# metarank/metarank

Hardware: AMD Instinct MI355X
Metric: ranked items/sec (feature assembly + 500-tree LambdaMART + ordering), Ranklens-shaped 100-item requests (higher is better)
Workload: dtype f64

## Files before the change

### metarank_amd/csrc/capi.cpp

```cpp
#include <cmath>
#include <cstddef>
#include <cstdlib>
#include <cstring>
#include <mutex>
#include <set>
#include <thread>
#include <utility>

#include "runtime.hpp"

namespace mrk {

static thread_local std::string g_last_error;
void set_last_error(const std::string &msg) { g_last_error = msg; }

static Switches read_switches() {
  Switches s;
  auto flag = [](const char *name, bool dflt) { const char *e = getenv(name); return e ? atoi(e) != 0 : dflt; };
  auto num = [](const char *name, int dflt) { const char *e = getenv(name); return e ? atoi(e) : dflt; };
  s.rank_fused = flag("MRK_RANK_FUSED", true);
  s.rank_cells = flag("MRK_RANK_CELLS", true);
  if (const char *e = getenv("MRK_SCORER")) s.scorer_walk = !strcmp(e, "walk");
  if (const char *e = getenv("MRK_FUSED_THREADS")) s.fused_threads = std::min(256, std::max(64, atoi(e) / 64 * 64));
  { const int fs = num("MRK_FUSED_SPLIT", 0); s.fused_split = fs == 1 || fs == 2 || fs == 4 ? fs : 0; }
// ... 25 lines not shown
  s.jit_shipped = flag("MRK_JIT_SHIPPED", true);
  if (const char *d = getenv("MRK_JIT_DEFINES")) s.jit_defines = d; else s.jit_defines.clear();
  s.thr_stage = flag("MRK_THR_STAGE", true);
  s.fused_lds_min = std::max(0, num("MRK_FUSED_LDS_MIN", 0));
  if (const char *d = getenv("MRK_JIT_CACHE_DIR")) s.jit_cache_dir = d;
  else if (const char *x = getenv("XDG_CACHE_HOME")) s.jit_cache_dir = std::string(x) + "/mrk_jit";
  else if (const char *h = getenv("HOME")) s.jit_cache_dir = std::string(h) + "/.cache/mrk_jit";
  if (s.jit_cache_dir == "off") s.jit_cache_dir.clear();
  s.big_sort_cap = num("MRK_BIG_SORT_CAP", 4096);
  s.big_sort_tile = num("MRK_BIG_SORT_TILE", 0);
  s.big_sort_bucket = num("MRK_BIG_SORT_BUCKET", 0);
  s.jit_prepass = flag("MRK_JIT_PREPASS", true);
  s.qs_split = num("MRK_QS_SPLIT", -1);
  s.qs_kernel = num("MRK_QS_KERNEL", 1);
  s.qs_byte = flag("MRK_QS_BYTE", true);
  s.qs_r = num("MRK_QS_R", 2);
  s.walk_tile = num("MRK_WALK_TILE", 0);
  s.encoder_graph = flag("MRK_ENCODER_GRAPH", false);
  s.encoder_skinny = num("MRK_ENCODER_SKINNY", 15);
  s.encoder_packed = flag("MRK_ENCODER_PACKED", true);
  s.encoder_f32_mfma = flag("MRK_ENCODER_F32_MFMA", true);
  return s;
}
static Switches &switches_storage() {
  static Switches s = read_switches();
  return s;
}
const Switches &switches() { return switches_storage(); }
void reload_switches() { switches_storage() = read_switches(); }

// ... 492 lines not shown
```

### metarank_amd/csrc/capi_rank.cpp

```cpp
#include <algorithm>
#include <atomic>
#include <chrono>
#include <condition_variable>
#include <cstring>
#include <thread>

#include <linux/futex.h>
#include <sched.h>
#include <sys/prctl.h>
#include <sys/syscall.h>
#include <time.h>
#include <unistd.h>

#include <cstdlib>

#include "features.hpp"
#include "jit.hpp"
#include "launch_shape.hpp"
#include "qs_device.hpp"
#include "rank.hpp"
#include "runtime.hpp"

namespace mrk {

// ... 64 lines not shown
}

}

using namespace mrk;

struct mrk_batch {
  mrk_ctx *ctx = nullptr;
  const Program *prog = nullptr;
  int n_req = 0, total_items = 0;
  std::mutex bmu;
  DevBuf d_in, d_prep_out, d_arena, d_matrix;
  hipStream_t stream = nullptr;
  hipStream_t s() const { return stream ? stream : ctx->stream; }
  DevBuf d_out;
  size_t out_order_off = 0, out_status_off = 0, out_bytes = 0;
  PinBuf h_out;
  bool fetch_enqueued = false;
  bool direct_out = false;
  DevBuf d_cells;
  DevBuf d_sort;
  DevBuf d_norm_order;
  DevBuf d_gather;
  DevBuf d_gather_status;
  struct BigReq { int r, n_items, item_begin; };
  std::vector<BigReq> big;
  PinBuf h_in;
  HostBatch hb;
  DevBuf d_ids;
  PinBuf h_ids;
  BatchDev view{};
// ... 117 lines not shown
  uint8_t *h = b.h_in.as<uint8_t>();
  auto put = [&](size_t o, const void *src, size_t bytes) { if (bytes) memcpy(h + o, src, bytes); };
  put(o_reqs, hb.reqs.data(), hb.reqs.size() * sizeof(ReqDev));
  put(o_consts, hb.consts.data(), hb.consts.size() * 8);
  put(o_irf, hb.irf.data(), hb.irf.size() * 4);
  put(o_ov, hb.overrides.data(), hb.overrides.size() * sizeof(Override));
  put(o_prep, hb.prep_out.data(), hb.prep_out.size() * sizeof(PrepOut));
  if (!hb.device_ids) {
    put(o_slot, hb.item_slot.data(), (size_t)T * 4);
    put(o_ireq, hb.item_req.data(), (size_t)T * 4);
  }
  MRK_HIP(hipMemcpyAsync(b.d_in.p, h, up_bytes, hipMemcpyHostToDevice, b.s()));
  uint8_t *d = b.d_in.as<uint8_t>();
  const size_t score_slots = (size_t)T + 256 * QS_TILE_ROWS;
  b.out_order_off = align_up(score_slots * 8, 256);
  b.out_status_off = align_up(b.out_order_off + std::max<size_t>(T, 1) * 4, 256);
  b.out_bytes = b.out_status_off + 2 * std::max<size_t>(n_req, 1) * 4;
  b.d_out.reserve(b.out_bytes);
  int32_t *d_load_status = (int32_t *)(b.d_out.as<uint8_t>() + b.out_status_off) + std::max(n_req, 1);
  MRK_HIP(hipMemsetAsync(d_load_status, 0, std::max<size_t>(n_req, 1) * 4, b.s()));
  if (hb.device_ids && T > 0) {
    const size_t off_bytes = ((size_t)T + 1) * 4;
    const size_t id_bytes = ids->offsets[T];
    if (id_bytes > ids->bytes_len || ids->bytes_len > 0xffffffffull)
      throw StatusError(MRK_ERR_INVALID_ARG, "mrk_item_ids: the last offset passes bytes_len (or bytes_len >= 4 GiB)");
    const size_t o_bytes = align_up(off_bytes, 256);
    b.d_ids.reserve(o_bytes + std::max<size_t>(id_bytes, 1));
    const void *src_off = ids->offsets, *src_bytes = ids->bytes;
    const bool own_staging = (const void *)ids->offsets == (const void *)b.h_ids.p;
    if (!own_staging && (!is_pinned_host(ids->offsets) || !is_pinned_host(ids->bytes))) {
      b.h_ids.reserve(o_bytes + std::max<size_t>(id_bytes, 1));
// ... 15 lines not shown
  v.total_items = T;
  v.item_lo = 0;
  v.item_hi = T;
  v.item_slot = (const int32_t *)(d + o_slot);
  v.item_req = (const uint32_t *)(d + o_ireq);
  v.consts = (const double *)(d + o_consts);
  v.irf = (const int32_t *)(d + o_irf);
  v.overrides = (const Override *)(d + o_ov);
  v.n_overrides = (int)hb.overrides.size();
  v.prep_out = (PrepOut *)(d + o_prep);
  v.arena = (unsigned long long *)b.d_arena.p;
  v.status = (int32_t *)(b.d_out.as<uint8_t>() + b.out_status_off);
  v.matrix = (double *)b.d_matrix.p;
  v.scores = (double *)b.d_out.p;
  v.order = (int32_t *)(b.d_out.as<uint8_t>() + b.out_order_off);
  b.h_status.assign(n_req, 0);
  b.ran = false;
  b.matrix_valid = false;
  b.fetch_enqueued = false;
  b.big.clear();
  size_t big_bytes = 0;
  for (int r = 0; r < n_req; ++r)
    if (hb.reqs[r].n_items > SORT_MAX_ITEMS) {
      b.big.push_back({r, hb.reqs[r].n_items, (int)hb.reqs[r].item_begin});
      big_bytes = std::max(big_bytes, big_sort_scratch_bytes(hb.reqs[r].n_items));
    }
  if (big_bytes) b.d_sort.reserve(big_bytes);
  uint32_t vals = 1;
  while ((int)vals < hb.max_doubles) vals <<= 1;
  b.fused_entries = (uint32_t)std::max<uint64_t>(hb.max_req_entries, 1);
// ... 95 lines not shown
  b.fetch_enqueued = false;
  b.direct_out = false;
  if (one) {
    b.h_out.reserve(b.out_bytes);
    uint8_t *h = b.h_out.as<uint8_t>();
    const OneOut out{(double *)h, (int32_t *)(h + b.out_order_off), (int32_t *)(h + b.out_status_off),
                     (const int32_t *)(b.d_out.as<uint8_t>() + b.out_status_off) + std::max(b.n_req, 1), std::max(b.n_req, 1)};
    b.view.item_lo = 0;
    b.view.item_hi = b.total_items;
    launch_rank_one(ctx, st, pd, b.view, b.fused_entries, b.fused_vals, b.fused_threads, b.fused_split, qs_device_view(model), qs_forest_view(model), out, f64, jit_fn);
    b.matrix_valid = false;
    b.direct_out = true;
    b.ran = true;
    return;
  }
  MRK_HIP(hipMemsetAsync(b.view.status, 0, std::max<size_t>(b.n_req, 1) * 4, b.s()));
  b.view.item_lo = whole_matrix ? 0 : lo;
  b.view.item_hi = whole_matrix ? b.total_items : hi;
  if (fused_score) {
    const QsDev q = qs_device_view(model);
    b.d_cells.reserve(std::max<size_t>((size_t)b.n_req * q.n_views * QS_TILE_ROWS * 2, 16));
    launch_rank_fused_score(ctx, st, pd, b.view, b.fused_entries, b.fused_vals, b.fused_threads, q, qs_forest_view(model), b.d_cells.as<uint16_t>(), f64, jit_fn);
    b.matrix_valid = false;
    b.ran = true;
    return;
  }
  if (cells) {
    const QsDev q = qs_device_view(model);
    const size_t tile_bytes = (size_t)q.n_views * QS_TILE_ROWS * 2;
    const size_t n_tiles = ((size_t)b.total_items + QS_TILE_ROWS - 1) / QS_TILE_ROWS;
    b.d_cells.reserve(std::max<size_t>(n_tiles * tile_bytes, 16));
    if (hi % QS_TILE_ROWS && tile_bytes)
      MRK_HIP(hipMemsetAsync(b.d_cells.as<uint8_t>() + (size_t)(hi / QS_TILE_ROWS) * tile_bytes, 0, tile_bytes, b.s()));
    if (b.fused_ok) {
      launch_rank_fused(ctx, st, pd, b.view, b.fused_entries, b.fused_vals, b.fused_threads, b.fused_split, b.fused_slices, &q, b.d_cells.as<uint16_t>(), f64, jit_fn,
                        sig && sig->ok ? (size_t)sig->rt_total * 8 : 0);
    } else {
      launch_prepass(ctx, st, pd, b.view, b.fused_entries, jit_prep_fn);
      launch_assemble_cells(ctx, st, pd, b.view, q, b.d_cells.as<uint16_t>(), f64, jit_fn, b.fused_entries, jit_rt_fn, jit_rt_fn ? model->qs_sig.rt_total : 0u);
    }
    b.matrix_valid = false;
    launch_score_qs_cells(ctx, model, b.d_cells.as<uint16_t>() + (size_t)(lo / QS_TILE_ROWS) * (tile_bytes / 2), rows, b.view.scores + lo);
  } else {
    assemble_matrix(b, st, pd, jit_fn);
    b.matrix_valid = whole_matrix || (lo == 0 && hi == b.total_items);
    if (model && rows > 0) {
      launch_score_batch(ctx, model, b.view.matrix + (size_t)lo * pd.dim, rows, pd.dim, b.view.scores + lo, b.view.status, b.view.item_req + lo);
    } else if (rows > 0) {
      MRK_HIP(hipMemsetAsync(b.view.scores + lo, 0, (size_t)rows * 8, b.s()));
    }
  }
  b.view.item_lo = 0;
  b.view.item_hi = b.total_items;
  if (sort) sort_batch(b);
  b.ran = true;
}

// ... 1331 lines not shown
```

### metarank_amd/csrc/rank.hip

```cpp
#include <hip/hip_runtime.h>

#include <cstdint>
#include <mutex>
#include <utility>

#include "rank_device.hpp"
#include "sort_device.hpp"
#include "runtime.hpp"

namespace mrk {

namespace {

__global__ void __launch_bounds__(PREP_THREADS)
prepass_kernel(StoreDev st, ProgramDev prog, BatchDev b, uint32_t lds_entries) { prepass_body(st, prog, b, lds_entries); }

__global__ void __launch_bounds__(ASM_THREADS)
assemble_kernel(StoreDev st, ProgramDev prog, BatchDev b) {
  const int gi0 = b.item_lo + blockIdx.x * ASM_THREADS + threadIdx.x;
  const bool active = gi0 < b.item_hi;
  if (!__any(active)) return;
  const int gi = active ? gi0 : b.item_hi - 1;
  const int r = (int)b.item_req[gi];
  const ReqDev rq = b.reqs[r];
// ... 46 lines not shown

template <bool F64>
__global__ void override_cells_kernel(BatchDev b, QsDev q, uint16_t *cells) {
  const int i = blockIdx.x * blockDim.x + threadIdx.x;
  if (i >= b.n_overrides) return;
  const Override o = b.overrides[i];
  if ((int)o.item < b.item_lo || (int)o.item >= b.item_hi) return;
  if ((int)o.col >= q.n_feats) return;
  const QsFeature ft = q.feats[o.col];
  uint16_t *d = cells + (size_t)(o.item / QS_TILE_ROWS) * q.n_views * QS_TILE_ROWS + (o.item % QS_TILE_ROWS);
  const bool ok = qs_bin_column<F64>(o.value, ft, q.views, q.thr, [d](uint32_t view, uint32_t cell) { d[view * QS_TILE_ROWS] = (uint16_t)cell; });
  if (!ok) atomicOr(&b.status[b.item_req[o.item]], 32);
}

constexpr int SORT_THREADS = 256;
constexpr int SORT_COUNT_MAX = 256;

__global__ void __launch_bounds__(SORT_THREADS)
sort_kernel(BatchDev b, int cap) {
  extern __shared__ __align__(16) unsigned long long sort_smem[];
  unsigned long long *s_key = sort_smem;
  int *s_idx = (int *)(sort_smem + cap);
  const int r = blockIdx.x;
  const int tid = threadIdx.x;
  const ReqDev rq = b.reqs[r];
  const int n = rq.n_items;
  if (n <= 0 || n > SORT_MAX_ITEMS) return;
  if (n <= SORT_COUNT_MAX) {
    for (int i = tid; i < n; i += SORT_THREADS) s_key[i] = sort_key(b.scores[rq.item_begin + i]);
    __syncthreads();
    for (int i = tid; i < n; i += SORT_THREADS) {
      const unsigned long long mine = s_key[i];
      int before = 0;
      for (int j = 0; j < n; ++j) {
        const unsigned long long kj = s_key[j];
        before += (kj < mine || (kj == mine && j < i)) ? 1 : 0;
      }
      b.order[rq.item_begin + before] = i;
    }
    return;
  }
  int p2 = 1;
  while (p2 < n) p2 <<= 1;
  for (int i = tid; i < p2; i += SORT_THREADS) {
    s_key[i] = i < n ? sort_key(b.scores[rq.item_begin + i]) : ~0ull;
    s_idx[i] = i < n ? i : 0x7fffffff;
  }
  __syncthreads();
  for (int k = 2; k <= p2; k <<= 1) {
    for (int j = k >> 1; j > 0; j >>= 1) {
      for (int p = tid; p < p2 / 2; p += SORT_THREADS) {
        const int i = ((p & ~(j - 1)) << 1) | (p & (j - 1)), ixj = i | j;
        const unsigned long long ka = s_key[i], kb = s_key[ixj];
        const int ia = s_idx[i], ib = s_idx[ixj];
// ... 328 lines not shown
```

### metarank_amd/csrc/rank.hpp

```cpp
#pragma once
#include "device_types.hpp"

namespace mrk {

enum OpKind : int32_t {
  OP_SCALAR_DOUBLE = 0,
  OP_SCALAR_BOOL = 1,
  OP_VECTOR = 2,
  OP_STRING_INDEX = 3,
  OP_STRING_ONEHOT = 4,
  OP_COUNTER = 5,
  OP_WINDOW = 6,
  OP_RATE = 7,
  OP_INTERACTED = 8,
  OP_DIVERSITY = 9,
  OP_ITEM_AGE = 10,
  OP_CONST = 11,
  OP_FILL_NAN = 12,
  OP_BIENCODER = 13,
};

enum RateMode : int32_t { RATE_ITEM = 0, RATE_ITEM_FIELD = 1, RATE_RANKING_FIELD = 2 };
enum NormMode : int32_t { NORM_NOOP = 0, NORM_MINMAX = 1, NORM_POSITION = 2 };

// ... 72 lines not shown
  int32_t n_req;
  int32_t total_items;
  int32_t item_lo, item_hi;
  const int32_t *item_slot;
  const uint32_t *item_req;
  const double *consts;
  const int32_t *irf;
  const Override *overrides;
  int32_t n_overrides;
  PrepOut *prep_out;
  unsigned long long *arena;
  int32_t *status;
  double *matrix;
  double *scores;
  int32_t *order;
};

constexpr int PREP_MAX_VALUES = 4096;
struct OneOut {
  double *scores;
  int32_t *order;
  int32_t *status;
  const int32_t *load_status;
  int32_t n_req_pad;
};

struct ServeCtl {
  uint32_t seq;
  uint32_t stop;
  uint32_t ack;
// ... 7 lines not shown
  ServeCtl *ctl;
  const uint8_t *in_host;
  uint8_t *in_dev;
  OneOut out;
};
constexpr int SERVE_GANG = 8;
struct ServeGangDev {
  const ServeSlotDev *slots;
  unsigned long long *clock;
  uint32_t launch_id, pad;
  unsigned long long idle_ticks;
  unsigned long long life_ticks;
};

constexpr int SORT_MAX_ITEMS = 4096;

}
```

### metarank_amd/csrc/rank_device.hpp

```cpp
#pragma once
#include <hip/hip_runtime.h>

#include "qs_device.hpp"
#include "rank.hpp"
#include "sort_device.hpp"
#include "table_device.hpp"
#include "wave_device.hpp"

#ifdef MRK_PHASE_CLOCKS
__device__ unsigned long long mrk_phase_clocks[64];
#define MRK_PHASE(prev, acc)                                                   \
  do {                                                                         \
    const unsigned long long t_ = clock64();                                   \
    (acc) += t_ - (prev);                                                      \
    (prev) = t_;                                                               \
  } while (0)
#else
#define MRK_PHASE(prev, acc) do { } while (0)
#endif

namespace mrk {

namespace {

// ... 1509 lines not shown
  const uint8_t *irec = record(st, SC_ITEM, islot);
  constexpr int NP = prog_item_pieces<Prog>(0);
  if constexpr (NP > 0 && NP <= REC_MAX_PIECES) {
    const RegRec<NP> ir = load_record_regs<NP>(irec);
    assemble_item_rec<SPLIT>(st, prog, b, gi, r, rq, tab_base, tab_sub, pos, sink, islot, ir, og, G);
  } else {
    const PtrRec ir{irec};
    assemble_item_rec<SPLIT>(st, prog, b, gi, r, rq, tab_base, tab_sub, pos, sink, islot, ir, og, G);
  }
}


template <bool SPLIT, typename Prog, typename SinkMaker>
__device__ __forceinline__ void rank_fused_body(const StoreDev &st, const Prog &prog, const BatchDev &b, uint32_t tab_entries,
                                                int vals_cap, uint32_t thr_cap, int mode, const SinkMaker &make_sink, uint32_t lds_skip = 0,
                                                const double *rt_src = nullptr, uint32_t rt_doubles = 0, int blk = -1) {
  const int op_split = SPLIT ? ((mode & 255) > 1 ? (mode & 255) : 1) : 1;
  const int slices = SPLIT ? (((mode >> 8) & 255) > 1 ? ((mode >> 8) & 255) : 1) : 1;
  extern __shared__ __align__(16) uint8_t smem_base[];
  uint8_t *smem = smem_base + lds_skip;
  unsigned long long *s_tab = (unsigned long long *)smem;
  double *s_vals = (double *)(smem + (size_t)tab_entries * 8);
  PrepOut *s_po = (PrepOut *)(smem + (size_t)tab_entries * 8 + (size_t)vals_cap * 8);
  int *s_int = (int *)(s_po + FUSED_MAX_PREP);
  const size_t thr_at = ((size_t)((uint8_t *)(s_int + PREP_INTS) - smem) + 15) & ~(size_t)15;
  qs_lds_double *s_thr_all = (qs_lds_double *)(smem + thr_at);
  qs_lds_double *s_thr = s_thr_all + (size_t)(threadIdx.x >> 6) * 2 * thr_cap;
  const int bid = blk < 0 ? (int)blockIdx.x : blk;
  const int r = bid / slices, sl = bid % slices;
  const ReqDev rq = b.reqs[r];
  if (rq.item_begin >= b.item_hi || rq.item_begin + rq.n_items <= b.item_lo) return;
  const int item_lanes = (int)blockDim.x / op_split;
  const int per = ((rq.n_items + slices - 1) / slices + item_lanes - 1) / item_lanes * item_lanes;
  const int slice_lo = sl * per, slice_hi = min(rq.n_items, slice_lo + per);
  if (sl > 0 && slice_lo >= rq.n_items) return;
  for (int e = threadIdx.x; e < prog.n_prep; e += blockDim.x) s_po[e] = b.prep_out[(size_t)r * prog.n_prep + e];
  if (rt_doubles) {
    const uint4 *src = (const uint4 *)rt_src;
    uint4 *dst = (uint4 *)(smem + thr_at);
    for (uint32_t i = threadIdx.x; i < rt_doubles / 2; i += blockDim.x) dst[i] = src[i];
  }
  __syncthreads();
  PrepScratch sc{s_vals, vals_cap, s_int, 0ull, {0, 0, 0, 0, 0, 0}};
#ifdef MRK_PHASE_CLOCKS
  sc.clk = clock64();
#endif
  prepass_request(st, prog, b, r, rq, s_tab, (uint32_t)rq.arena_begin, s_po, sc);
  const int og = (int)threadIdx.x / item_lanes, il = (int)threadIdx.x % item_lanes;
  for (int base = slice_lo; base < slice_hi; base += item_lanes) {
    const int i = base + il;
// ... 122 lines not shown
    atomicAdd(&mrk_phase_clocks[5], clk_acc[1]);
    atomicAdd(&mrk_phase_clocks[6], 1ull);
  }
#endif
}

template <bool SPLIT = false, typename Prog>
__device__ __forceinline__ void rank_fused_matrix_body(const StoreDev &st, const Prog &prog, const BatchDev &b, uint32_t tab_entries, int vals_cap, int mode = 1) {
  rank_fused_body<SPLIT>(st, prog, b, tab_entries, vals_cap, 0u, mode,
                  [&](int gi, int, bool active, qs_lds_double *, qs_lds_double *) { return MatrixSink{b.matrix + (size_t)gi * prog.dim, active}; });
}

template <bool F64, bool SPLIT = false, typename QS = QsDyn, typename Prog>
__device__ __forceinline__ void rank_fused_cells_body(const StoreDev &st, const Prog &prog, const BatchDev &b, uint32_t tab_entries,
                                                      int vals_cap, const QsDev &q, uint16_t *cells, int mode = 1) {
  if constexpr (qs_fused_rt<QS, SPLIT>()) {
    rank_fused_body<SPLIT>(st, prog, b, tab_entries, vals_cap, qs_thr_cap<QS>(q), mode, [&](int gi, int r, bool active, qs_lds_double *, qs_lds_double *s_all) {
      return CellSinkRT<F64, QS, !SPLIT>{q, cells + (size_t)(gi / QS_TILE_ROWS) * QS::n_views * QS_TILE_ROWS + (gi % QS_TILE_ROWS), &b.status[r], s_all, active};
    }, 0u, q.thr_rt, QS::rt_total);
  } else {
    rank_fused_body<SPLIT>(st, prog, b, tab_entries, vals_cap, qs_thr_cap<QS>(q), mode, [&](int gi, int r, bool active, qs_lds_double *s_thr, qs_lds_double *) {
      return CellSink<F64, QS>{q, cells + (size_t)(gi / QS_TILE_ROWS) * qs_n_views<QS>(q) * QS_TILE_ROWS + (gi % QS_TILE_ROWS), &b.status[r], s_thr, active};
    });
  }
}

template <bool F64, typename QS = QsDyn, typename Prog>
__device__ __forceinline__ void rank_one_body(const StoreDev &st, const Prog &prog, const BatchDev &b, uint32_t tab_entries, int vals_cap,
                                              const QsDev &q, const QsForestDev &f, int mode, const OneOut &out, int blk = -1) {
  extern __shared__ __align__(16) uint8_t smem_base[];
  const int tid = threadIdx.x, nthr = blockDim.x;
  const int r = blk < 0 ? (int)blockIdx.x : blk;
  const ReqDev rq = b.reqs[r];
  const uint32_t slab_bytes = (uint32_t)qs_n_views<QS>(q) * (QS_TILE_ROWS * 2);
  for (uint32_t i = tid; i < slab_bytes / 4 + 4; i += nthr) ((uint32_t *)smem_base)[i] = 0u;
  int32_t *s_status = (int32_t *)(smem_base + slab_bytes);
  BatchDev bl = b;
  bl.status = s_status - r;
// ... 181 lines not shown
```

### metarank_amd/csrc/runtime.hpp

```cpp
#pragma once
#include <hip/hip_runtime.h>

#include <atomic>
#include <condition_variable>
#include <cstdint>
#include <map>
#include <memory>
#include <mutex>
#include <shared_mutex>
#include <stdexcept>
#include <string>
#include <vector>

#include "../../include/mrk.h"
#include "forest.hpp"

namespace mrk {

struct StatusError : std::runtime_error {
  int status;
  StatusError(int s, const std::string &m) : std::runtime_error(m), status(s) {}
};

void set_last_error(const std::string &msg);
// ... 101 lines not shown
  bool items_lds = true;
  int rank_one_max = 128;
  int split_max_req = 64;
  bool items_rt = true;
  int items_rt_threads = 0;
  bool jit_sig = true;
  bool jit_record_regs = true;
  std::string jit_cache_dir;
  int big_sort_cap = 4096;
  bool jit_prepass = true;
  int big_sort_bucket = 0;
  int big_sort_tile = 0;
  int qs_split = -1;
  int qs_kernel = 1;
  bool qs_byte = true;
  int qs_r = 2;
  int walk_tile = 0;
  bool encoder_graph = false;
  int encoder_skinny = 15;
  bool encoder_packed = true;
  bool encoder_f32_mfma = true;
};
const Switches &switches();
void reload_switches();


}

struct mrk_ctx {
  std::atomic<int> refs{1};
// ... 73 lines not shown

void lds_optin(mrk_ctx *ctx, const void *fn, int bytes = 160 * 1024);

int hw_queue_budget();

void ctx_retain(mrk_ctx *ctx);
void ctx_release(mrk_ctx *ctx);

void free_rank_state(mrk_ctx *ctx);
void comm_destroy(mrk_ctx *ctx);
void comm_allgather_f64_inplace(mrk_ctx *ctx, double *buf, size_t chunk, hipStream_t stream);
void comm_allgather_f64(mrk_ctx *ctx, const double *send, double *recv, size_t count, hipStream_t stream);
void comm_allgather_i32(mrk_ctx *ctx, const int32_t *send, int32_t *recv, size_t count, hipStream_t stream);
void unbind_encoders(mrk_ctx *ctx);

void launch_score(mrk_ctx *ctx, mrk_model *m, const double *d_x, int rows, int cols, double *d_out,
                  int *d_flag);
uint32_t score_chunk_budget();
bool launch_score_qs(mrk_ctx *ctx, mrk_model *m, const double *d_x, int rows, int cols, double *d_out, int *d_flag,
                     const uint32_t *d_row_req);
void launch_score_qs_cells(mrk_ctx *ctx, mrk_model *m, const uint16_t *d_cells, int rows, double *d_out);

}
```

### metarank_amd/csrc/score_qs.hip

```cpp
#include <hip/hip_runtime.h>

#include <algorithm>
#include <cstdint>
#include <cstdlib>

#include "launch_shape.hpp"
#include "qs_device.hpp"
#include "runtime.hpp"

namespace mrk {

QsDev qs_device_view(const mrk_model *m);

namespace {

constexpr int QS_WAVES = 4;


template <bool F64>
__global__ void __launch_bounds__(256)
qs_bin_kernel(const double *__restrict__ X, int rows, int cols, QsDev q, uint16_t *__restrict__ cells, int tile_rows,
              long long padded_rows, int *__restrict__ flag, const uint32_t *__restrict__ row_req) {
  const long long row = (long long)blockIdx.x * 256 + threadIdx.x;
  if (row >= padded_rows) return;
// ... 223 lines not shown
#pragma unroll
    for (int j = 0; j < R; ++j) { if constexpr (F64) acc64[j] += lb64[j]; else acc32[j] += lb32[j]; }
  }
#pragma unroll
  for (int j = 0; j < R; ++j) { if constexpr (F64) acc64[j] += la64[j]; else acc32[j] += la32[j]; }
  if (!odd) {
#pragma unroll
    for (int j = 0; j < R; ++j) { if constexpr (F64) acc64[j] += lb64[j]; else acc32[j] += lb32[j]; }
  }
  const long long row0 = tile * (R * 64) + (long long)lane * R;
#pragma unroll
  for (int j = 0; j < R; ++j)
    if (row0 + j < rows) out[row0 + j] = F64 ? acc64[j] : (double)acc32[j];
}

template <bool F64, int NW>
__global__ void __launch_bounds__(NW * 64)
qs_score_split_kernel(const uint32_t *__restrict__ nodes, const uint8_t *__restrict__ leaves,
                      const QsCatNode *__restrict__ cat_nodes, const uint32_t *__restrict__ cat_bits,
                      const uint16_t *__restrict__ cells, int n_trees, int V, int rows, double base,
                      double *__restrict__ out) {
  constexpr int LS = F64 ? 8 : 4;
  constexpr int TREE_LEAF_BYTES = QS_LEAVES * LS;
  constexpr int CH = 8 * NW;
  extern __shared__ __align__(16) uint8_t smem[];
  uint8_t *s_leaf = smem + (size_t)V * 256;
  uint8_t *s_idx = s_leaf + CH * TREE_LEAF_BYTES;
  const int tid = threadIdx.x;
  const int lane = tid & 63;
  const int wave = __builtin_amdgcn_readfirstlane(tid >> 6);
  const long long tile = blockIdx.x;
  {
    const uint4 *src = (const uint4 *)(cells + (size_t)tile * V * QS_TILE_ROWS);
    uint4 *dst = (uint4 *)smem;
    for (int i = tid; i < V * 16; i += NW * 64) dst[i] = src[i];
  }
// ... 42 lines not shown
      }
      const uint32_t inv = ~accn;
      const uint32_t pair = (uint32_t)__builtin_ctz(inv) | ((uint32_t)__builtin_ctz(inv >> 16) << 8);
      *(uint16_t *)(s_idx + tt * QS_TILE_ROWS + lane * 2) = (uint16_t)pair;
    }
    __syncthreads();
    if (tid < QS_TILE_ROWS) {
      for (int tt = 0; tt < nt; ++tt) {
        const uint32_t li = s_idx[tt * QS_TILE_ROWS + tid];
        if constexpr (F64) acc64 += *(const double *)(s_leaf + tt * TREE_LEAF_BYTES + li * 8);
        else acc32 += *(const float *)(s_leaf + tt * TREE_LEAF_BYTES + li * 4);
      }
    }
  }
  const long long row = tile * QS_TILE_ROWS + tid;
  if (tid < QS_TILE_ROWS && row < rows) out[row] = F64 ? acc64 : (double)acc32;
}

template <int B0>
__device__ __forceinline__ void qs_byte_block(uint32_t &acc, const uint32_t (&d)[QS_SLOTS - 1], const uint32_t (&m)[QS_SLOTS]) {
#pragma unroll
  for (int s = B0; s < B0 + 4 && s < QS_SLOTS - 1; ++s) asm("v_and_or_b32 %0, %1, %2, %0" : "+v"(acc) : "v"(d[s]), "s"(m[s]));
}

template <bool F64, int NW>
__global__ void __launch_bounds__(NW * 64)
qs_score_byte_split_kernel(const uint32_t *__restrict__ bnodes, const uint8_t *__restrict__ leaves,
                           const QsCatNode *__restrict__ cat_nodes, const uint32_t *__restrict__ cat_bits,
                           const uint16_t *__restrict__ cells, int n_trees, int V, int rows, double base,
                           double *__restrict__ out) {
  constexpr int LS = F64 ? 8 : 4;
  constexpr int TREE_LEAF_BYTES = QS_LEAVES * LS;
  constexpr int CH = 8 * NW;
  extern __shared__ __align__(16) uint8_t smem[];
  uint8_t *s_leaf = smem + (size_t)V * 256;
  uint8_t *s_idx = s_leaf + CH * TREE_LEAF_BYTES;
  const int tid = threadIdx.x;
  const int lane = tid & 63;
  const int wave = __builtin_amdgcn_readfirstlane(tid >> 6);
  const long long tile = blockIdx.x;
  const uint16_t *tile_cells = cells + (size_t)tile * V * QS_TILE_ROWS;
  {
    const uint4 *src = (const uint4 *)tile_cells;
    uint4 *dst = (uint4 *)smem;
    typedef unsigned short ushort2v __attribute__((ext_vector_type(2)));
// ... 59 lines not shown
      }
      const uint32_t inv = ~accn;
      const uint32_t pair = (uint32_t)__builtin_ctz(inv) | ((uint32_t)__builtin_ctz(inv >> 16) << 8);
      *(uint16_t *)(s_idx + tt * QS_TILE_ROWS + lane * 2) = (uint16_t)pair;
    }
    __syncthreads();
    if (tid < QS_TILE_ROWS) {
      for (int tt = 0; tt < nt; ++tt) {
        const uint32_t li = s_idx[tt * QS_TILE_ROWS + tid];
        if constexpr (F64) acc64 += *(const double *)(s_leaf + tt * TREE_LEAF_BYTES + li * 8);
        else acc32 += *(const float *)(s_leaf + tt * TREE_LEAF_BYTES + li * 4);
      }
    }
  }
  const long long row = tile * QS_TILE_ROWS + tid;
  if (tid < QS_TILE_ROWS && row < rows) out[row] = F64 ? acc64 : (double)acc32;
}

template <bool F64>
void launch_wave(mrk_ctx *ctx, mrk_model *m, const uint16_t *d_cells, int rows, double *d_out) {
  const PackedForestQS &q = m->qs;
  const int V = (int)q.views.size();
  const long long n_tiles = ((long long)rows + QS_TILE_ROWS - 1) / QS_TILE_ROWS;
  const int split_env = switches().qs_split;
  const int nw = split_env >= 0 ? split_env : scorer_waves_per_tile(n_tiles, V, F64, ctx->n_cus, QS_LEAVES, QS_TILE_ROWS);
  if (nw == 2 || nw == 4 || nw == 8 || nw == 16) {
    const size_t lds = (size_t)V * 256 + (size_t)8 * nw * (QS_LEAVES * (F64 ? 8 : 4) + QS_TILE_ROWS);
    if (lds <= 160 * 1024) {
      ScopedKernelTimer timer(ctx, "score");
      const bool byte_mode = q.byte_ok && switches().qs_byte;
#define MRK_SPLIT(NW_)                                                                                                      \
      {                                                                                                                       \
        auto sk = byte_mode ? qs_score_byte_split_kernel<F64, NW_> : qs_score_split_kernel<F64, NW_>;                        \
        lds_optin(ctx, (const void *)sk);                                                                                     \
        hipLaunchKernelGGL(sk, dim3((unsigned)n_tiles), dim3(NW_ * 64), lds, ctx->launch,                                     \
                           byte_mode ? m->d_qs_bnodes.as<uint32_t>() : m->d_qs_nodes.as<uint32_t>(),                          \
                           m->d_qs_leaves.as<uint8_t>(), m->d_qs_catnodes.as<QsCatNode>(), m->d_qs_cat.as<uint32_t>(), d_cells, \
                           q.n_trees, V, rows, m->forest.base_score, d_out);                                                  \
      }
      if (nw == 16) MRK_SPLIT(16) else if (nw == 8) MRK_SPLIT(8) else if (nw == 4) MRK_SPLIT(4) else MRK_SPLIT(2)
#undef MRK_SPLIT
      MRK_HIP(hipGetLastError());
      return;
    }
  }
  auto wk = qs_score_wave_kernel<F64>;
  lds_optin(ctx, (const void *)wk);
  const size_t lds = (size_t)V * 256;
  ScopedKernelTimer timer(ctx, "score");
  hipLaunchKernelGGL(wk, dim3((unsigned)n_tiles), dim3(64), lds, ctx->launch, m->d_qs_nodes.as<uint32_t>(),
                     m->d_qs_leaves.as<uint8_t>(), m->d_qs_catnodes.as<QsCatNode>(), m->d_qs_cat.as<uint32_t>(), d_cells,
                     q.n_trees, V, rows, m->forest.base_score, d_out);
  MRK_HIP(hipGetLastError());
}

template <bool F64, int R>
void launch_generic(mrk_ctx *ctx, mrk_model *m, const uint16_t *d_cells, int rows, double *d_out, int chunk_trees, size_t smem) {
  const PackedForestQS &q = m->qs;
  const int V = (int)q.views.size();
  const long long n_tiles = ((long long)rows + R * 64 - 1) / (R * 64);
  auto kern = qs_score_kernel<F64, R>;
  lds_optin(ctx, (const void *)kern);
  ScopedKernelTimer timer(ctx, "score");
  const int grid = (int)((n_tiles + QS_WAVES - 1) / QS_WAVES);
  hipLaunchKernelGGL(kern, dim3(grid), dim3(QS_WAVES * 64), smem, ctx->launch, m->d_qs_nodes.as<uint32_t>(),
                     m->d_qs_leaves.as<uint8_t>(), m->d_qs_catnodes.as<QsCatNode>(), m->d_qs_cat.as<uint32_t>(), d_cells,
                     q.n_trees, V, rows, n_tiles, m->forest.base_score, d_out, chunk_trees);
  MRK_HIP(hipGetLastError());
// ... 58 lines not shown
  f.cat_nodes = m->d_qs_catnodes.as<QsCatNode>();
  f.cat_bits = m->d_qs_cat.as<uint32_t>();
  f.n_trees = m->qs.n_trees;
  f.n_views = (int32_t)m->qs.views.size();
  f.base = m->forest.base_score;
  return f;
}

bool launch_score_qs(mrk_ctx *ctx, mrk_model *m, const double *d_x, int rows, int cols, double *d_out, int *d_flag,
                     const uint32_t *d_row_req) {
  if (!m->qs.ok) return false;
  if (m->forest.backend == Backend::LightGBM) return launch_qs_b<true>(ctx, m, d_x, rows, cols, d_out, d_flag, d_row_req);
  return launch_qs_b<false>(ctx, m, d_x, rows, cols, d_out, d_flag, d_row_req);
}

void launch_score_qs_cells(mrk_ctx *ctx, mrk_model *m, const uint16_t *d_cells, int rows, double *d_out) {
  if (m->forest.backend == Backend::LightGBM) launch_wave<true>(ctx, m, d_cells, rows, d_out);
  else launch_wave<false>(ctx, m, d_cells, rows, d_out);
}

}
```

### metarank_amd/csrc/sort_device.hpp

```cpp
#pragma once
#include <hip/hip_runtime.h>

#include <cstdint>

namespace mrk {

__device__ __forceinline__ unsigned long long asc_key(double v) {
  unsigned long long bits = (unsigned long long)__double_as_longlong(v);
  if (v != v) bits = 0x7ff8000000000000ULL;
  return (bits & 0x8000000000000000ULL) ? ~bits : (bits | 0x8000000000000000ULL);
}
__device__ __forceinline__ double asc_value(unsigned long long key) {
  const unsigned long long bits = (key & 0x8000000000000000ULL) ? (key & 0x7fffffffffffffffULL) : ~key;
  return __longlong_as_double((long long)bits);
}
__device__ __forceinline__ unsigned long long sort_key(double score) { return asc_key(-score); }

__device__ __forceinline__ bool pair_lt(unsigned long long ka, int ia, unsigned long long kb, int ib) {
  return ka < kb || (ka == kb && ia < ib);
}

struct SortSrc {
  const double *vals;
  const unsigned long long *raw;
  long long stride;
  int negate;
};
__device__ __forceinline__ unsigned long long src_key(const SortSrc &s, int i) {
  if (s.raw) return s.raw[i];
  const double v = s.vals[(long long)i * s.stride];
  return s.negate ? sort_key(v) : asc_key(v);
}

}
```

Measured before the change: 1.103 billion.

## Fuse per-request ordering into QS scorer epilogue behind opt-in switch

Adds an optional epilogue to the split QuickScorer kernels. Each tile counting-sorts the requests that lie wholly inside it. For requests that span tiles, an atomic arrival counter lets the last tile to finish sort the whole request, so the separate sort kernel launch is skipped. It also moves the status/arrival clearing into the fused assembly kernel when it owns a whole request, which drops a memset. The reordering is gated by MRK_SCORE_ORDER, off by default, but the owner-clears memset removal and the count_order refactor of sort_kernel do run by default.

Measured after the change: 1.088 billion. -1.4%, worse.

```diff
diff --git a/metarank_amd/csrc/capi.cpp b/metarank_amd/csrc/capi.cpp
--- a/metarank_amd/csrc/capi.cpp
+++ b/metarank_amd/csrc/capi.cpp
@@ -63,6 +63,7 @@
   s.qs_split = num("MRK_QS_SPLIT", -1);
   s.qs_kernel = num("MRK_QS_KERNEL", 1);
   s.qs_byte = flag("MRK_QS_BYTE", true);
+  s.score_order = flag("MRK_SCORE_ORDER", false);
   s.qs_r = num("MRK_QS_R", 2);
   s.walk_tile = num("MRK_WALK_TILE", 0);
   s.encoder_graph = flag("MRK_ENCODER_GRAPH", false);
diff --git a/metarank_amd/csrc/capi_rank.cpp b/metarank_amd/csrc/capi_rank.cpp
--- a/metarank_amd/csrc/capi_rank.cpp
+++ b/metarank_amd/csrc/capi_rank.cpp
@@ -102,7 +102,7 @@
   hipStream_t stream = nullptr;
   hipStream_t s() const { return stream ? stream : ctx->stream; }
   DevBuf d_out;
-  size_t out_order_off = 0, out_status_off = 0, out_bytes = 0;
+  size_t out_order_off = 0, out_arrive_off = 0, out_status_off = 0, out_bytes = 0;
   PinBuf h_out;
   bool fetch_enqueued = false;
   bool direct_out = false;
@@ -250,7 +250,8 @@
   uint8_t *d = b.d_in.as<uint8_t>();
   const size_t score_slots = (size_t)T + 256 * QS_TILE_ROWS;
   b.out_order_off = align_up(score_slots * 8, 256);
-  b.out_status_off = align_up(b.out_order_off + std::max<size_t>(T, 1) * 4, 256);
+  b.out_arrive_off = align_up(b.out_order_off + std::max<size_t>(T, 1) * 4, 256);
+  b.out_status_off = b.out_arrive_off + std::max<size_t>(n_req, 1) * 4;
   b.out_bytes = b.out_status_off + 2 * std::max<size_t>(n_req, 1) * 4;
   b.d_out.reserve(b.out_bytes);
   int32_t *d_load_status = (int32_t *)(b.d_out.as<uint8_t>() + b.out_status_off) + std::max(n_req, 1);
@@ -296,6 +297,7 @@
   v.matrix = (double *)b.d_matrix.p;
   v.scores = (double *)b.d_out.p;
   v.order = (int32_t *)(b.d_out.as<uint8_t>() + b.out_order_off);
+  v.arrive = (uint32_t *)(b.d_out.as<uint8_t>() + b.out_arrive_off);
   b.h_status.assign(n_req, 0);
   b.ran = false;
   b.matrix_valid = false;
@@ -421,7 +423,10 @@
     b.ran = true;
     return;
   }
-  MRK_HIP(hipMemsetAsync(b.view.status, 0, std::max<size_t>(b.n_req, 1) * 4, b.s()));
+  const bool whole = lo == 0 && hi == b.total_items;
+  const bool score_order = sort && sw.score_order && cells && !fused_score && whole && b.hb.max_items <= SORT_COUNT_MAX && b.big.empty();
+  const bool owner_clears = cells && !fused_score && whole && b.fused_ok && b.fused_split == 1 && b.fused_slices == 1;
+  if (!owner_clears) MRK_HIP(hipMemsetAsync(b.view.arrive, 0, 2 * std::max<size_t>(b.n_req, 1) * 4, b.s()));
   b.view.item_lo = whole_matrix ? 0 : lo;
   b.view.item_hi = whole_matrix ? b.total_items : hi;
   if (fused_score) {
@@ -447,7 +452,9 @@
       launch_assemble_cells(ctx, st, pd, b.view, q, b.d_cells.as<uint16_t>(), f64, jit_fn, b.fused_entries, jit_rt_fn, jit_rt_fn ? model->qs_sig.rt_total : 0u);
     }
     b.matrix_valid = false;
-    launch_score_qs_cells(ctx, model, b.d_cells.as<uint16_t>() + (size_t)(lo / QS_TILE_ROWS) * (tile_bytes / 2), rows, b.view.scores + lo);
+    if (launch_score_qs_cells(ctx, model, b.d_cells.as<uint16_t>() + (size_t)(lo / QS_TILE_ROWS) * (tile_bytes / 2), rows, b.view.scores + lo,
+                              score_order ? &b.view : nullptr))
+      sort = false;
   } else {
     assemble_matrix(b, st, pd, jit_fn);
     b.matrix_valid = whole_matrix || (lo == 0 && hi == b.total_items);
diff --git a/metarank_amd/csrc/rank.hip b/metarank_amd/csrc/rank.hip
--- a/metarank_amd/csrc/rank.hip
+++ b/metarank_amd/csrc/rank.hip
@@ -84,7 +84,6 @@
 }
 
 constexpr int SORT_THREADS = 256;
-constexpr int SORT_COUNT_MAX = 256;
 
 __global__ void __launch_bounds__(SORT_THREADS)
 sort_kernel(BatchDev b, int cap) {
@@ -99,15 +98,7 @@
   if (n <= SORT_COUNT_MAX) {
     for (int i = tid; i < n; i += SORT_THREADS) s_key[i] = sort_key(b.scores[rq.item_begin + i]);
     __syncthreads();
-    for (int i = tid; i < n; i += SORT_THREADS) {
-      const unsigned long long mine = s_key[i];
-      int before = 0;
-      for (int j = 0; j < n; ++j) {
-        const unsigned long long kj = s_key[j];
-        before += (kj < mine || (kj == mine && j < i)) ? 1 : 0;
-      }
-      b.order[rq.item_begin + before] = i;
-    }
+    count_order<1>(s_key, n, tid, SORT_THREADS, b.order + rq.item_begin);
     return;
   }
   int p2 = 1;
diff --git a/metarank_amd/csrc/rank.hpp b/metarank_amd/csrc/rank.hpp
--- a/metarank_amd/csrc/rank.hpp
+++ b/metarank_amd/csrc/rank.hpp
@@ -110,6 +110,7 @@
   double *matrix;
   double *scores;
   int32_t *order;
+  uint32_t *arrive;
 };
 
 constexpr int PREP_MAX_VALUES = 4096;
@@ -147,5 +148,6 @@
 };
 
 constexpr int SORT_MAX_ITEMS = 4096;
+constexpr int SORT_COUNT_MAX = 256;
 
 }
diff --git a/metarank_amd/csrc/rank_device.hpp b/metarank_amd/csrc/rank_device.hpp
--- a/metarank_amd/csrc/rank_device.hpp
+++ b/metarank_amd/csrc/rank_device.hpp
@@ -1547,7 +1547,8 @@
 template <bool SPLIT, typename Prog, typename SinkMaker>
 __device__ __forceinline__ void rank_fused_body(const StoreDev &st, const Prog &prog, const BatchDev &b, uint32_t tab_entries,
                                                 int vals_cap, uint32_t thr_cap, int mode, const SinkMaker &make_sink, uint32_t lds_skip = 0,
-                                                const double *rt_src = nullptr, uint32_t rt_doubles = 0, int blk = -1) {
+                                                const double *rt_src = nullptr, uint32_t rt_doubles = 0, int blk = -1,
+                                                bool own_status = false) {
   const int op_split = SPLIT ? ((mode & 255) > 1 ? (mode & 255) : 1) : 1;
   const int slices = SPLIT ? (((mode >> 8) & 255) > 1 ? ((mode >> 8) & 255) : 1) : 1;
   extern __shared__ __align__(16) uint8_t smem_base[];
@@ -1567,6 +1568,10 @@
   const int per = ((rq.n_items + slices - 1) / slices + item_lanes - 1) / item_lanes * item_lanes;
   const int slice_lo = sl * per, slice_hi = min(rq.n_items, slice_lo + per);
   if (sl > 0 && slice_lo >= rq.n_items) return;
+  if (own_status && threadIdx.x == 0) {
+    b.status[r] = 0;
+    b.arrive[r] = 0u;
+  }
   for (int e = threadIdx.x; e < prog.n_prep; e += blockDim.x) s_po[e] = b.prep_out[(size_t)r * prog.n_prep + e];
   if (rt_doubles) {
     const uint4 *src = (const uint4 *)rt_src;
@@ -1719,14 +1724,15 @@
 template <bool F64, bool SPLIT = false, typename QS = QsDyn, typename Prog>
 __device__ __forceinline__ void rank_fused_cells_body(const StoreDev &st, const Prog &prog, const BatchDev &b, uint32_t tab_entries,
                                                       int vals_cap, const QsDev &q, uint16_t *cells, int mode = 1) {
+  const bool own = !SPLIT || ((mode & 255) <= 1 && ((mode >> 8) & 255) <= 1);
   if constexpr (qs_fused_rt<QS, SPLIT>()) {
     rank_fused_body<SPLIT>(st, prog, b, tab_entries, vals_cap, qs_thr_cap<QS>(q), mode, [&](int gi, int r, bool active, qs_lds_double *, qs_lds_double *s_all) {
       return CellSinkRT<F64, QS, !SPLIT>{q, cells + (size_t)(gi / QS_TILE_ROWS) * QS::n_views * QS_TILE_ROWS + (gi % QS_TILE_ROWS), &b.status[r], s_all, active};
-    }, 0u, q.thr_rt, QS::rt_total);
+    }, 0u, q.thr_rt, QS::rt_total, -1, own);
   } else {
     rank_fused_body<SPLIT>(st, prog, b, tab_entries, vals_cap, qs_thr_cap<QS>(q), mode, [&](int gi, int r, bool active, qs_lds_double *s_thr, qs_lds_double *) {
       return CellSink<F64, QS>{q, cells + (size_t)(gi / QS_TILE_ROWS) * qs_n_views<QS>(q) * QS_TILE_ROWS + (gi % QS_TILE_ROWS), &b.status[r], s_thr, active};
-    });
+    }, 0u, nullptr, 0u, -1, own);
   }
 }
 
diff --git a/metarank_amd/csrc/runtime.hpp b/metarank_amd/csrc/runtime.hpp
--- a/metarank_amd/csrc/runtime.hpp
+++ b/metarank_amd/csrc/runtime.hpp
@@ -139,6 +139,7 @@
   int qs_split = -1;
   int qs_kernel = 1;
   bool qs_byte = true;
+  bool score_order = false;
   int qs_r = 2;
   int walk_tile = 0;
   bool encoder_graph = false;
@@ -242,11 +243,13 @@
 void comm_allgather_i32(mrk_ctx *ctx, const int32_t *send, int32_t *recv, size_t count, hipStream_t stream);
 void unbind_encoders(mrk_ctx *ctx);
 
+struct BatchDev;
+
 void launch_score(mrk_ctx *ctx, mrk_model *m, const double *d_x, int rows, int cols, double *d_out,
                   int *d_flag);
 uint32_t score_chunk_budget();
 bool launch_score_qs(mrk_ctx *ctx, mrk_model *m, const double *d_x, int rows, int cols, double *d_out, int *d_flag,
                      const uint32_t *d_row_req);
-void launch_score_qs_cells(mrk_ctx *ctx, mrk_model *m, const uint16_t *d_cells, int rows, double *d_out);
+bool launch_score_qs_cells(mrk_ctx *ctx, mrk_model *m, const uint16_t *d_cells, int rows, double *d_out, const mrk::BatchDev *order_view = nullptr);
 
 }
diff --git a/metarank_amd/csrc/score_qs.hip b/metarank_amd/csrc/score_qs.hip
--- a/metarank_amd/csrc/score_qs.hip
+++ b/metarank_amd/csrc/score_qs.hip
@@ -6,7 +6,9 @@
 
 #include "launch_shape.hpp"
 #include "qs_device.hpp"
+#include "rank.hpp"
 #include "runtime.hpp"
+#include "sort_device.hpp"
 
 namespace mrk {
 
@@ -261,12 +263,83 @@
     if (row0 + j < rows) out[row0 + j] = F64 ? acc64[j] : (double)acc32[j];
 }
 
+struct QsOrderDev {
+  const ReqDev *reqs;
+  const uint32_t *item_req;
+  int32_t *order;
+  uint32_t *arrive;
+};
+constexpr uint32_t QS_ORDER_LDS = SORT_COUNT_MAX * 8 + 16;
+
+template <int NTHR>
+__device__ __forceinline__ void qs_order_epilogue(const QsOrderDev &o, uint8_t *smem, long long tile, int rows, double score,
+                                                  const double *out) {
+  static_assert(NTHR % 64 == 0 && NTHR >= QS_TILE_ROWS, "two lanes per row in whole trips");
+  unsigned long long *s_key = (unsigned long long *)smem;
+  uint32_t *s_last = (uint32_t *)(smem + SORT_COUNT_MAX * 8);
+  const int tid = threadIdx.x;
+  const long long row_lo = tile * QS_TILE_ROWS;
+  const int n_rows = (int)min((long long)QS_TILE_ROWS, rows - row_lo);
+  __syncthreads();
+  if (tid < QS_TILE_ROWS) s_key[tid] = sort_key(score);
+  const int r_first = (int)o.item_req[row_lo], r_last = (int)o.item_req[row_lo + n_rows - 1];
+  const ReqDev rq_first = o.reqs[r_first], rq_last = o.reqs[r_last];
+  const int strad_r[2] = {r_first, r_last};
+  const int strad_b[2] = {rq_first.item_begin, rq_last.item_begin}, strad_n[2] = {rq_first.n_items, rq_last.n_items};
+  const bool strad[2] = {order_tile_arrives(rq_first.item_begin, rq_first.n_items, row_lo, QS_TILE_ROWS),
+                         r_last != r_first && order_tile_arrives(rq_last.item_begin, rq_last.n_items, row_lo, QS_TILE_ROWS)};
+  asm volatile("s_waitcnt vmcnt(0)" ::: "memory");
+  __syncthreads();
+  if (tid == 0) {
+    uint32_t last[2] = {0u, 0u};
+    if (strad[0] || strad[1]) {
+      __builtin_amdgcn_fence(__ATOMIC_RELEASE, "agent");
+      asm volatile("s_waitcnt vmcnt(0)" ::: "memory");
+#pragma unroll
+      for (int k = 0; k < 2; ++k)
+        if (strad[k]) {
+          const uint32_t seen = __hip_atomic_fetch_add(o.arrive + strad_r[k], 1u, __ATOMIC_RELAXED, __HIP_MEMORY_SCOPE_AGENT);
+          last[k] = seen + 1u == (uint32_t)order_arrivals(strad_b[k], strad_n[k], QS_TILE_ROWS) && strad_n[k] <= SORT_COUNT_MAX;
+        }
+      if (last[0] | last[1]) {
+        __builtin_amdgcn_fence(__ATOMIC_ACQUIRE, "agent");
+        asm volatile("s_waitcnt vmcnt(0)" ::: "memory");
+      }
+    }
+    s_last[0] = last[0];
+    s_last[1] = last[1];
+  }
+  for (int e = tid; e < 2 * QS_TILE_ROWS; e += NTHR) {
+    const int row = e >> 1, p = e & 1;
+    const bool valid = row < n_rows;
+    const int r = (int)o.item_req[row_lo + (valid ? row : 0)];
+    const ReqDev rq = o.reqs[r];
+    const bool whole = valid && rq.item_begin >= row_lo && (long long)rq.item_begin + rq.n_items <= row_lo + QS_TILE_ROWS;
+    const int k0 = whole ? (int)(rq.item_begin - row_lo) : 0, n = whole ? rq.n_items : 0;
+    int before = n ? count_part<2>(s_key + k0, n, row - k0, p) : 0;
+    before += __shfl_xor(before, 1);
+    if (whole && p == 0) o.order[rq.item_begin + before] = row - k0;
+  }
+  __syncthreads();
+  const bool last0 = s_last[0] != 0u, last1 = s_last[1] != 0u;
+  if (!(last0 | last1)) return;
+#pragma unroll
+  for (int k = 0; k < 2; ++k) {
+    if (!(k == 0 ? last0 : last1)) continue;
+    const int n = strad_n[k];
+    if (k == 1 && last0) __syncthreads();
+    for (int i = tid; i < n; i += NTHR) s_key[i] = sort_key(out[strad_b[k] + i]);
+    __syncthreads();
+    count_order<2>(s_key, n, tid, NTHR, o.order + strad_b[k]);
+  }
+}
+
 template <bool F64, int NW>
 __global__ void __launch_bounds__(NW * 64)
 qs_score_split_kernel(const uint32_t *__restrict__ nodes, const uint8_t *__restrict__ leaves,
                       const QsCatNode *__restrict__ cat_nodes, const uint32_t *__restrict__ cat_bits,
                       const uint16_t *__restrict__ cells, int n_trees, int V, int rows, double base,
-                      double *__restrict__ out) {
+                      double *out, QsOrderDev ord) {
   constexpr int LS = F64 ? 8 : 4;
   constexpr int TREE_LEAF_BYTES = QS_LEAVES * LS;
   constexpr int CH = 8 * NW;
@@ -339,7 +412,9 @@
     }
   }
   const long long row = tile * QS_TILE_ROWS + tid;
-  if (tid < QS_TILE_ROWS && row < rows) out[row] = F64 ? acc64 : (double)acc32;
+  const double score = F64 ? acc64 : (double)acc32;
+  if (tid < QS_TILE_ROWS && row < rows) out[row] = score;
+  if (ord.reqs) qs_order_epilogue<NW * 64>(ord, smem, tile, rows, score, out);
 }
 
 template <int B0>
@@ -353,7 +428,7 @@
 qs_score_byte_split_kernel(const uint32_t *__restrict__ bnodes, const uint8_t *__restrict__ leaves,
                            const QsCatNode *__restrict__ cat_nodes, const uint32_t *__restrict__ cat_bits,
                            const uint16_t *__restrict__ cells, int n_trees, int V, int rows, double base,
-                           double *__restrict__ out) {
+                           double *out, QsOrderDev ord) {
   constexpr int LS = F64 ? 8 : 4;
   constexpr int TREE_LEAF_BYTES = QS_LEAVES * LS;
   constexpr int CH = 8 * NW;
@@ -443,11 +518,13 @@
     }
   }
   const long long row = tile * QS_TILE_ROWS + tid;
-  if (tid < QS_TILE_ROWS && row < rows) out[row] = F64 ? acc64 : (double)acc32;
+  const double score = F64 ? acc64 : (double)acc32;
+  if (tid < QS_TILE_ROWS && row < rows) out[row] = score;
+  if (ord.reqs) qs_order_epilogue<NW * 64>(ord, smem, tile, rows, score, out);
 }
 
 template <bool F64>
-void launch_wave(mrk_ctx *ctx, mrk_model *m, const uint16_t *d_cells, int rows, double *d_out) {
+bool launch_wave(mrk_ctx *ctx, mrk_model *m, const uint16_t *d_cells, int rows, double *d_out, const BatchDev *order_view = nullptr) {
   const PackedForestQS &q = m->qs;
   const int V = (int)q.views.size();
   const long long n_tiles = ((long long)rows + QS_TILE_ROWS - 1) / QS_TILE_ROWS;
@@ -455,7 +532,10 @@
   const int nw = split_env >= 0 ? split_env : scorer_waves_per_tile(n_tiles, V, F64, ctx->n_cus, QS_LEAVES, QS_TILE_ROWS);
   if (nw == 2 || nw == 4 || nw == 8 || nw == 16) {
     const size_t lds = (size_t)V * 256 + (size_t)8 * nw * (QS_LEAVES * (F64 ? 8 : 4) + QS_TILE_ROWS);
+    static_assert(QS_ORDER_LDS <= 8 * 2 * (QS_LEAVES * 4 + QS_TILE_ROWS), "the epilogue's keys fit the smallest split kernel's dead areas");
     if (lds <= 160 * 1024) {
+      QsOrderDev ord{nullptr, nullptr, nullptr, nullptr};
+      if (order_view) ord = QsOrderDev{order_view->reqs, order_view->item_req, order_view->order, order_view->arrive};
       ScopedKernelTimer timer(ctx, "score");
       const bool byte_mode = q.byte_ok && switches().qs_byte;
 #define MRK_SPLIT(NW_)                                                                                                      \
@@ -465,12 +545,12 @@
         hipLaunchKernelGGL(sk, dim3((unsigned)n_tiles), dim3(NW_ * 64), lds, ctx->launch,                                     \
                            byte_mode ? m->d_qs_bnodes.as<uint32_t>() : m->d_qs_nodes.as<uint32_t>(),                          \
                            m->d_qs_leaves.as<uint8_t>(), m->d_qs_catnodes.as<QsCatNode>(), m->d_qs_cat.as<uint32_t>(), d_cells, \
-                           q.n_trees, V, rows, m->forest.base_score, d_out);                                                  \
+                           q.n_trees, V, rows, m->forest.base_score, d_out, ord);                                             \
       }
       if (nw == 16) MRK_SPLIT(16) else if (nw == 8) MRK_SPLIT(8) else if (nw == 4) MRK_SPLIT(4) else MRK_SPLIT(2)
 #undef MRK_SPLIT
       MRK_HIP(hipGetLastError());
-      return;
+      return order_view != nullptr;
     }
   }
   auto wk = qs_score_wave_kernel<F64>;
@@ -481,6 +561,7 @@
                      m->d_qs_leaves.as<uint8_t>(), m->d_qs_catnodes.as<QsCatNode>(), m->d_qs_cat.as<uint32_t>(), d_cells,
                      q.n_trees, V, rows, m->forest.base_score, d_out);
   MRK_HIP(hipGetLastError());
+  return false;
 }
 
 template <bool F64, int R>
@@ -569,9 +650,9 @@
   return launch_qs_b<false>(ctx, m, d_x, rows, cols, d_out, d_flag, d_row_req);
 }
 
-void launch_score_qs_cells(mrk_ctx *ctx, mrk_model *m, const uint16_t *d_cells, int rows, double *d_out) {
-  if (m->forest.backend == Backend::LightGBM) launch_wave<true>(ctx, m, d_cells, rows, d_out);
-  else launch_wave<false>(ctx, m, d_cells, rows, d_out);
-}
-
-}
+bool launch_score_qs_cells(mrk_ctx *ctx, mrk_model *m, const uint16_t *d_cells, int rows, double *d_out, const BatchDev *order_view) {
+  if (m->forest.backend == Backend::LightGBM) return launch_wave<true>(ctx, m, d_cells, rows, d_out, order_view);
+  return launch_wave<false>(ctx, m, d_cells, rows, d_out, order_view);
+}
+
+}
diff --git a/metarank_amd/csrc/sort_device.hpp b/metarank_amd/csrc/sort_device.hpp
--- a/metarank_amd/csrc/sort_device.hpp
+++ b/metarank_amd/csrc/sort_device.hpp
@@ -1,5 +1,7 @@
 #pragma once
+#ifndef MRK_SORT_HOST_TEST
 #include <hip/hip_runtime.h>
+#endif
 
 #include <cstdint>
 
@@ -20,6 +22,42 @@
   return ka < kb || (ka == kb && ia < ib);
 }
 
+
+__device__ __forceinline__ int count_before(const unsigned long long *keys, int j0, int j1, unsigned long long mine, int i) {
+  int before = 0;
+  for (int j = j0; j < j1; ++j) {
+    const unsigned long long kj = keys[j];
+    before += (kj < mine || (kj == mine && j < i)) ? 1 : 0;
+  }
+  return before;
+}
+template <int PARTS>
+__device__ __forceinline__ int count_part(const unsigned long long *keys, int n, int i, int p) {
+  return count_before(keys, (int)((long long)p * n / PARTS), (int)((long long)(p + 1) * n / PARTS), keys[i], i);
+}
+template <int PARTS>
+__device__ __forceinline__ void count_order(const unsigned long long *keys, int n, int t, int lanes, int32_t *out) {
+  static_assert(PARTS == 1 || PARTS == 2, "lanes per candidate");
+  for (int e = t; e < n * PARTS; e += lanes) {
+    const int i = e / PARTS, p = e % PARTS;
+    int before = count_part<PARTS>(keys, n, i, p);
+    if constexpr (PARTS == 2) before += __shfl_xor(before, 1);
+    if (p == 0) out[before] = i;
+  }
+}
+
+__device__ __forceinline__ int order_tiles_touched(int item_begin, int n_items, int tile_rows) {
+  return n_items <= 0 ? 0 : (item_begin + n_items - 1) / tile_rows - item_begin / tile_rows + 1;
+}
+__device__ __forceinline__ int order_arrivals(int item_begin, int n_items, int tile_rows) {
+  const int t = order_tiles_touched(item_begin, n_items, tile_rows);
+  return t > 1 ? t : 0;
+}
+__device__ __forceinline__ bool order_tile_arrives(int item_begin, int n_items, long long row_lo, int tile_rows) {
+  const long long lo = item_begin, hi = (long long)item_begin + n_items;
+  return n_items > 0 && lo < row_lo + tile_rows && hi > row_lo && (lo < row_lo || hi > row_lo + tile_rows);
+}
+
 struct SortSrc {
   const double *vals;
   const unsigned long long *raw;
```
